# kkromberg/SpeechRecognition

Measured on AMD Instinct MI355X. Metric: frames/sec scored+decoded, higher is better.
Workload: dtype f64

## Files before the change

### include/srgpu.h

```cpp
#ifndef SRGPU_H
#define SRGPU_H

#include <stddef.h>
#include <stdint.h>

#ifdef __cplusplus
extern "C" {
#endif

#if defined(__GNUC__)
#define SR_API __attribute__((visibility("default")))
#else
#define SR_API
#endif

#define SR_ABI_VERSION 4
SR_API int sr_abi_version(void);

#define SR_OK 0
#define SR_EINVAL (-1)
#define SR_EHIP (-2)
#define SR_ENODEV (-3)
#define SR_ELIMIT (-4)
#define SR_ENOMEM (-5)
// ... 263 lines not shown
                                 sr_bigram_stream** out);
SR_API int sr_bigram_stream_begin(sr_bigram_stream* s, uint32_t* id);
SR_API int sr_bigram_stream_push(sr_bigram_stream* s, uint32_t n, const uint32_t* ids, const float* feats, const uint64_t* frame_off);
SR_API int sr_bigram_stream_partial(sr_bigram_stream* s, uint32_t id, uint32_t* out_word, float* out_score, uint32_t* out_time,
                                    uint32_t cap, uint32_t* count, uint64_t* frames);
SR_API int sr_bigram_stream_end(sr_bigram_stream* s, uint32_t id, uint32_t* out_word, float* out_score, uint32_t* out_time,
                                uint32_t cap, uint32_t* count);
SR_API int sr_bigram_stream_destroy(sr_bigram_stream* s);

SR_API int sr_probe_fp16_denormals(int device, int* preserved);
SR_API int sr_probe_fp16_accumulation(int device, int* within_model, double* worst_ratio);

SR_API int sr_prefilter_masks(sr_model* m, const float* feats, uint64_t n_frames, int route, uint32_t* n_groups, uint32_t* masks,
                              uint64_t cap_words);
SR_API int sr_prefilter_range_frames(uint32_t* frames);

typedef struct {
  double gmm_ms;
  uint64_t gmm_launches;
  double gmm_flops;
  double search_ms;
  uint64_t search_launches;
  double search_bytes;
  uint64_t frames;
  uint64_t refined_pairs;
  uint64_t refined_densities;
  double prefilter_ms;
  double refine_ms;
} sr_profile;
SR_API int sr_profile_enable(sr_model* m, int on);
// ... 8 lines not shown
```

### speechrecognition_amd/build.py

```python
from __future__ import annotations

import hashlib
import os
import subprocess
import sys

HERE = os.path.dirname(os.path.abspath(__file__))
CSRC = os.path.join(HERE, "csrc")
LIB = os.path.join(HERE, "libsrgpu.so")
SOURCES = ["srgpu_api.cpp", "mixset.cpp", "feeder.cpp", "gmm_mfma.hip", "gmm_exact.hip", "gmm_prefilter.hip", "viterbi_decode.hip",
           "viterbi_fast.hip", "viterbi_words.hip", "viterbi_align.hip", "viterbi_fb.hip", "viterbi_netfb.hip", "viterbi_mmi.hip", "viterbi_smbr.hip", "viterbi_lattice.hip", "viterbi_bigram.hip", "viterbi_bigram_fb.hip", "viterbi_bigram_mmi.hip", "viterbi_bigram_smbr.hip", "viterbi_bigram_lattice.hip", "posterior_items.hip",
           "em_accumulate.hip", "em_finalize.hip", "fmllr_stats.hip", "fmllr.cpp", "mllr_stats.hip", "mllt_stats.hip", "lda_stats.hip", "model_structure.hip"]
HEADERS = ["mllr.cpp", "mllt.cpp", "lda.cpp", "kernels.h", "host_util.h", "handles.h", "traceback.h", "dpp_util.h", "netfb_device.h", "smbr_device.h", "sym_contract.h", "structure_plan.h", "fb_plan.h", os.path.join("..", "..", "include", "srgpu.h")]
FLAGS = ["-O3", "-std=c++17", "--offload-arch=gfx950", "-fPIC", "-fvisibility=hidden", "-Wall", "-Wno-unused-function"]
PER_FILE = {"gmm_exact.hip": ["-ffp-contract=off"], "gmm_prefilter.hip": ["-ffp-contract=off"], "em_accumulate.hip": ["-ffp-contract=off"],
            "em_finalize.hip": ["-ffp-contract=off"],
            "viterbi_bigram_lattice.hip": ["-ffp-contract=off"],
            "fmllr_stats.hip": ["-ffp-contract=off"],
            "mllr_stats.hip": ["-ffp-contract=off"],
            "mllt_stats.hip": ["-ffp-contract=off"],
            "lda_stats.hip": ["-ffp-contract=off"],
            "model_structure.hip": ["-ffp-contract=off"]}
MAX_PARALLEL = 8


def _read(path):
    with open(path, "rb") as f:
# ... 115 lines not shown
```

### speechrecognition_amd/capi.py

```python
from __future__ import annotations

import ctypes as C
import os

import numpy as np

HERE = os.path.dirname(os.path.abspath(__file__))
LIB_PATH = os.environ.get("SRGPU_LIB") or os.path.join(HERE, "libsrgpu.so")

GMM_MFMA, GMM_EXACT, GMM_PREFILTER, GMM_DEFAULT = 0, 1, 2, 3
POOL_GLOBAL, POOL_MIXTURE, POOL_NONE = 0, 1, 2
SEARCH_GENERAL_KERNEL = 1
SEARCH_SLOT_KERNEL = 2
BIGRAM_DENSE_STATES = 1
BIGRAM_GLOBAL_STATES = 2
SR_ECORRUPT = -7
LDA_SKIP = 0xFFFFFFFF
SR_ABI_VERSION = 4

SYMBOLS = [
    "sr_abi_version", "sr_model_trim",
    "sr_last_error", "sr_device_count", "sr_model_create", "sr_model_load_mixset", "sr_model_destroy", "sr_model_info",
    "sr_corpus_upload", "sr_corpus_upload_async", "sr_corpus_wait", "sr_corpus_destroy", "sr_shard_utterances", "sr_recognize_batch_multi", "sr_score_corpus", "sr_score_frames", "sr_lexicon_create",
    "sr_lexicon_destroy", "sr_lexicon_describe", "sr_recognize_corpus", "sr_traceback_corpus", "sr_traceback_words", "sr_recognize_batch", "sr_align_corpus", "sr_align_corpus_pruned", "sr_path_scores_corpus", "sr_model_create_from_statistics", "sr_model_create_from_accumulated", "sr_mixset_write", "sr_model_set_tying", "sr_model_tying_info", "sr_model_topology", "sr_accumulate_corpus",
# ... 3 lines not shown
    "sr_smbr_max_positions", "sr_net_accuracies_corpus", "sr_smbr_statistics_corpus",
    "sr_word_lattice_corpus", "sr_lattice_nbest",
    "sr_fmllr_statistics_corpus", "sr_fmllr_statistics_bw_corpus", "sr_fmllr_estimate", "sr_corpus_transform",
    "sr_mllr_statistics_corpus", "sr_mllr_statistics_bw_corpus", "sr_mllr_estimate", "sr_model_transform_means",
    "sr_mllt_statistics_corpus", "sr_mllt_statistics_bw_corpus", "sr_mllt_estimate",
    "sr_lda_statistics_corpus", "sr_lda_estimate", "sr_corpus_splice_transform",
    "sr_bigram_create", "sr_bigram_destroy", "sr_bigram_describe", "sr_recognize_bigram_corpus",
    "sr_bigram_word_posteriors_corpus", "sr_recognize_bigram_confidence_corpus",
    "sr_bigram_occupancies_corpus", "sr_bigram_mmi_statistics_corpus",
    "sr_bigram_accuracies_corpus", "sr_bigram_smbr_statistics_corpus",
    "sr_bigram_word_lattice_corpus", "sr_bigram_lattice_nbest",
    "sr_stream_open", "sr_stream_begin", "sr_stream_push", "sr_stream_partial", "sr_stream_end", "sr_stream_destroy",
    "sr_bigram_stream_open", "sr_bigram_stream_begin", "sr_bigram_stream_push", "sr_bigram_stream_partial", "sr_bigram_stream_end",
    "sr_bigram_stream_destroy",
    "sr_probe_fp16_denormals", "sr_probe_fp16_accumulation", "sr_prefilter_masks", "sr_prefilter_range_frames",
    "sr_profile_enable", "sr_profile_reset", "sr_profile_read",
]


class SrError(RuntimeError):
    def __init__(self, code, msg):
        super().__init__(f"libsrgpu error {code}: {msg}")
        self.code = code


def prefilter_range_frames():
    n = C.c_uint32()
    _check(lib().sr_prefilter_range_frames(C.byref(n)))
    return n.value

# ... 109 lines not shown
        L.sr_stream_begin.argtypes = [vp, C.POINTER(u32)]
        L.sr_stream_push.argtypes = [vp, u32, vp, vp, vp]
        L.sr_stream_partial.argtypes = [vp, u32, vp, u32, C.POINTER(u32), C.POINTER(u64)]
        L.sr_stream_end.argtypes = [vp, u32, vp, u32, C.POINTER(u32), vp, vp, vp]
        L.sr_stream_destroy.argtypes = [vp]
        L.sr_bigram_stream_open.argtypes = [vp, vp, C.POINTER(BigramParams), u32, u64, C.POINTER(vp)]
        L.sr_bigram_stream_begin.argtypes = [vp, C.POINTER(u32)]
        L.sr_bigram_stream_push.argtypes = [vp, u32, vp, vp, vp]
        L.sr_bigram_stream_partial.argtypes = [vp, u32, vp, vp, vp, u32, C.POINTER(u32), C.POINTER(u64)]
        L.sr_bigram_stream_end.argtypes = [vp, u32, vp, vp, vp, u32, C.POINTER(u32)]
        L.sr_bigram_stream_destroy.argtypes = [vp]
        L.sr_probe_fp16_denormals.argtypes = [i32, C.POINTER(i32)]
        L.sr_probe_fp16_accumulation.argtypes = [i32, C.POINTER(i32), C.POINTER(dbl)]
        L.sr_prefilter_masks.argtypes = [vp, vp, u64, i32, C.POINTER(u32), vp, u64]
        L.sr_prefilter_range_frames.argtypes = [C.POINTER(u32)]
        L.sr_profile_enable.argtypes = [vp, i32]
        L.sr_profile_reset.argtypes = [vp]
        L.sr_profile_read.argtypes = [vp, C.POINTER(Profile)]
        _lib = L
    return _lib


def _check(rc):
    if rc != 0:
        raise SrError(rc, lib().sr_last_error().decode(errors="replace"))


def device_count():
    n = C.c_int(0)
    _check(lib().sr_device_count(C.byref(n)))
# ... 112 lines not shown
        self.close()

    def score_frames(self, feats, kernel=GMM_PREFILTER):
        feats = np.ascontiguousarray(feats, dtype=np.float32)
        out = np.empty((feats.shape[0], self.n_states), dtype=np.float64)
        _check(lib().sr_score_frames(self.h, _ptr(feats), feats.shape[0], kernel, _ptr(out)))
        return out

    def prefilter_masks(self, feats, route):
        feats = np.ascontiguousarray(feats, dtype=np.float32)
        n_groups = C.c_uint32()
        _check(lib().sr_prefilter_masks(self.h, None, feats.shape[0], route, C.byref(n_groups), None, 0))
        out = np.empty((n_groups.value, feats.shape[0], 4), dtype=np.uint32)
        _check(lib().sr_prefilter_masks(self.h, _ptr(feats), feats.shape[0], route, C.byref(n_groups), _ptr(out), out.size))
        return out

    def upload(self, feats, frame_off, asynchronous=False):
        return Corpus(self, feats, frame_off, asynchronous)

    def recognize_batch(self, lexicon, feats, frame_off, am_threshold, word_penalty, kernel=GMM_PREFILTER):
        feats = np.ascontiguousarray(feats, dtype=np.float32)
        frame_off = np.ascontiguousarray(frame_off, dtype=np.uint64)
        n = len(frame_off) - 1
        words = np.zeros(max(int(frame_off[-1]), 1), dtype=np.uint32)
        woff = np.zeros(n + 1, dtype=np.uint64)
        sp = SearchParams(am_threshold, word_penalty, kernel, 0)
        _check(lib().sr_recognize_batch(self.h, lexicon.h, C.byref(sp), _ptr(feats), _ptr(frame_off), n, _ptr(words), _ptr(woff)))
        return words[: int(woff[-1])].copy(), woff

    def lexicon(self, word_off, automaton, silence_idx, tdp, silence_state):
# ... 728 lines not shown
```

### speechrecognition_amd/csrc/handles.h

```cpp
#pragma once
#include <hip/hip_runtime.h>

#include <atomic>
#include <condition_variable>
#include <cstdint>
#include <map>
#include <memory>
#include <mutex>
#include <string>
#include <thread>
#include <vector>

#include "../../include/srgpu.h"
#include "host_util.h"
#include "kernels.h"

namespace srhost {
int fail(int code, const char* fmt, ...) __attribute__((format(printf, 2, 3)));
}

#define HIP_TRY(expr)                                                                             \
  do {                                                                                            \
    hipError_t e_ = (expr);                                                                       \
    if (e_ != hipSuccess) return srhost::fail(SR_EHIP, "%s: %s (%s:%d)", #expr, hipGetErrorString(e_), __FILE__, __LINE__); \
// ... 12 lines not shown
    return e;
  }
  hipError_t upload(const T* src, size_t count) {
    hipError_t e = ensure(count);
    if (e != hipSuccess || count == 0) return e;
    return hipMemcpy(p, src, count * sizeof(T), hipMemcpyHostToDevice);
  }
  void release() { if (p) (void)hipFree(p); p = nullptr; n = 0; }
  void swap(DevBuf& o) { T* tp = p; p = o.p; o.p = tp; size_t tn = n; n = o.n; o.n = tn; }
  DevBuf() = default;
  DevBuf(const DevBuf&) = delete;
  DevBuf& operator=(const DevBuf&) = delete;
  ~DevBuf() { release(); }
};

struct EventPair { hipEvent_t a, b; int kind; };


struct sr_feeder;


struct CorpusSpare {
  DevBuf<float> feats;
  DevBuf<uint64_t> d_frame_off;
  DevBuf<uint32_t> utt_order, out_words, out_count, out_flags;
  DevBuf<double> tb_score;
  DevBuf<uint16_t> tb_word, tb_bkp;
  size_t bytes() const {
    return feats.n * 4 + d_frame_off.n * 8 + (utt_order.n + out_words.n + out_count.n + out_flags.n) * 4 + tb_score.n * 8 + (tb_word.n + tb_bkp.n) * 2;
  }
};
size_t corpus_spare_cap_bytes();

struct sr_model {
  int device = 0;
  uint32_t dim = 0, n_states = 0, ld = 0;
  uint64_t n_dens = 0;
  bool max_approx = true;
  DevBuf<uint32_t> dens_off;
  DevBuf<double> means, inv_vars, norm, logw;
  DevBuf<uint32_t> dens_mean, dens_var;
  std::vector<uint32_t> h_dens_off, h_dens_mean, h_dens_var;
  std::vector<double> h_means, h_inv_vars, h_norm, h_logw;
  bool mfma_packed = false, pf_packed = false;
// ... 6 lines not shown
  std::map<uint32_t, std::unique_ptr<DevBuf<uint32_t>>> split_tabs, pf_split_tabs;
  const uint32_t *split_cur = nullptr, *pf_split_cur = nullptr;
  uint32_t split_ny = 0;
  int pf_ks32 = 0;
  uint32_t pf_groups = 0, pf_ny = 0, max_dens = 0, pf_slots = 0, pf_chunks = 1, pf_pstates = 0;
  DevBuf<unsigned char> pf_apack;
  DevBuf<float> pf_lim, featsT, featsP;
  DevBuf<uint4> pf_defer;
  DevBuf<uint32_t> pf_defer_cnt;
  int neg_possible = -1;
  uint32_t pf_dp = 0;
  DevBuf<uint32_t> pf_mask, pf_ndens, pf_ring;
  DevBuf<uint4> pf_bfrag;
  DevBuf<float2> pf_bnorm;
  int pf_route = srgpu::kPfStationary;
  DevBuf<double> pf_rows;
  DevBuf<unsigned long long> pf_counter;
  hipStream_t s_copy = nullptr;
  float* staging[2] = {nullptr, nullptr};
  hipEvent_t staging_free[2] = {nullptr, nullptr};
  std::atomic<bool> staging_busy{false};
  std::mutex spare_mu;
  std::unique_ptr<CorpusSpare> spare;
  std::vector<sr_corpus*> corpora;
  hipStream_t s_gmm = nullptr, s_search = nullptr;
  DevBuf<double> scores[2];
  hipEvent_t ev_scored[2] = {nullptr, nullptr}, ev_consumed[2] = {nullptr, nullptr};
  size_t chunk_frames = 0;
  bool overlap = true;
  size_t defer_budget = (size_t)32 << 30;
// ... 7 lines not shown
};

struct sr_corpus {
  sr_model* model = nullptr;
  sr_feeder* feeder = nullptr;
  uint32_t n_utts = 0;
  uint64_t n_frames = 0;
  std::vector<uint64_t> frame_off;
  DevBuf<float> feats;
  DevBuf<uint64_t> d_frame_off;
  DevBuf<uint32_t> utt_order;
  size_t order_chunk_frames = 0;
  DevBuf<double> tb_score;
  DevBuf<uint16_t> tb_word, tb_bkp;
  DevBuf<uint32_t> out_words, out_count, out_flags;
  DevBuf<unsigned char> big_ws;
  DevBuf<uint16_t> automata, out_states;
  DevBuf<uint64_t> aut_off, bp_off, al_blk_frame0;
  DevBuf<uint32_t> al_list_off, al_states, al_blk_frames, al_blk_list;
  DevBuf<uint8_t> backptr;
  DevBuf<double> out_cost, path_scores;
  DevBuf<uint64_t> pair_off;
  DevBuf<uint32_t> pair_frame, key_mean, key_var, iota, keys_sorted, pairs_sorted, row_begin;
  DevBuf<double> pair_w, acc_mean, acc_var, w_mean, w_var;
  bool acc_valid = false;
  uint32_t acc_n_mean = 0, acc_n_var = 0;
  DevBuf<unsigned char> sort_temp;
  DevBuf<double> fb_trellis, fb_item_w, fb_weight;
  DevBuf<uint64_t> fb_trellis_off, fb_pair_cnt, fb_pair_end;
  DevBuf<uint32_t> fb_mix_off, fb_slot_beg, fb_cnt, fb_scan, fb_base, fb_item_off, fb_item_frame;
// ... 144 lines not shown
```

### speechrecognition_amd/csrc/kernels.h

```cpp
#pragma once
#include <hip/hip_runtime.h>
#include <stdint.h>

#include <vector>

namespace srgpu {

struct GmmMfmaArgs {
  const float* feats;
  uint64_t n_frames;
  uint32_t dim;
  const double* apack;
  const uint32_t* blk_meta;
  const uint32_t* grp_state;
  const uint32_t* split_begin;
  double* out;
  uint32_t ld;
  uint32_t nx, ny;
};
int gmm_mfma_ksteps_for_dim(uint32_t dim);
int gmm_mfma_frames_per_tile(int ksteps);
hipError_t launch_gmm_mfma(const GmmMfmaArgs& a, int ksteps, bool sum, hipStream_t stream);

struct GmmExactArgs {
// ... 175 lines not shown
  const StreamJob* jobs;
  unsigned char* ws;
  size_t ws_stride;
  StreamState* state;
  double* tb_score;
  uint16_t* tb_word;
  uint16_t* tb_bkp;
  uint64_t tb_stride;
  uint32_t* words;
  uint64_t words_stride;
};
hipError_t launch_decode_stream(const StreamArgs& a, uint32_t n_jobs, hipStream_t stream);
hipError_t launch_traceback(const uint64_t* frame_off, uint32_t n_utts, const uint16_t* tb_word, const uint16_t* tb_bkp,
                            uint32_t silence_word, uint32_t n_words, uint32_t* out_words, uint32_t* out_count,
                            uint32_t* out_flags, hipStream_t stream);

struct AlignArgs {
  const double* scores;
  uint32_t ld;
  const uint64_t* frame_off;
  uint64_t frame_base;
  uint32_t utt_first, n_utts;
  const uint32_t* utt_order;
  const uint16_t* automata;
  const uint64_t* aut_off;
  double tdp_loop, tdp_forward, tdp_skip;
  uint32_t silence_state;
  double pruning_threshold;
  uint8_t* backptr;
  const uint64_t* bp_off;
// ... 447 lines not shown
```

### speechrecognition_amd/csrc/srgpu_api.cpp

```cpp
#include <hip/hip_runtime.h>

#include <algorithm>
#include <cmath>
#include <cstdarg>
#include <cstdio>
#include <cstdlib>
#include <cstring>
#include <limits>
#include <map>
#include <memory>
#include <mutex>
#include <numeric>
#include <queue>
#include <set>
#include <string>
#include <vector>

#include "../../include/srgpu.h"
#include "fb_plan.h"
#include "host_util.h"
#include "kernels.h"
#include "traceback.h"

using namespace srgpu;
// ... 493 lines not shown
    if ((rc = launch_scoring(m, c->feats.p + a * m->dim, cuts[i] - a, gmm_kernel, table + (a - f0) * m->ld))) return rc;
    a = cuts[i];
  }
  return SR_OK;
}

int prepare_chunks(sr_model* m, sr_corpus* c, std::vector<Chunk>* chunks) {
  *chunks = make_chunks(c, m->chunk_frames);
  uint64_t mx = 0;
  for (const Chunk& ch : *chunks) mx = std::max(mx, ch.f1 - ch.f0);
  const int nbuf = chunks->size() > 1 ? 2 : 1;
  for (int i = 0; i < nbuf; i++) HIP_TRY(m->scores[i].ensure((size_t)mx * m->ld));
  return ensure_utt_order(m, c, *chunks);
}

template <class Score, class Search>
int run_chunks(sr_model* m, const std::vector<Chunk>& chunks, Score score, Search search) {
  const hipStream_t s_search = m->overlap ? m->s_search : m->s_gmm;
  int rc;
  for (size_t i = 0; i < chunks.size(); i++) {
    const int buf = (int)(i & 1);
    if (i >= 2) HIP_TRY(hipStreamWaitEvent(m->s_gmm, m->ev_consumed[buf], 0));
    if ((rc = score(chunks[i], m->scores[buf].p))) return rc;
    HIP_TRY(hipEventRecord(m->ev_scored[buf], m->s_gmm));
    HIP_TRY(hipStreamWaitEvent(s_search, m->ev_scored[buf], 0));
    EventPair ep{};
    if ((rc = prof_begin(m, s_search, 1, &ep))) return rc;
    if ((rc = search(chunks[i], m->scores[buf].p, s_search))) return rc;
    if ((rc = prof_end(m, s_search, &ep))) return rc;
    HIP_TRY(hipEventRecord(m->ev_consumed[buf], s_search));
  }
  HIP_TRY(hipStreamSynchronize(m->s_search));
  HIP_TRY(hipStreamSynchronize(m->s_gmm));
  return SR_OK;
}

}
namespace srhost {
static void swap_spare(sr_corpus* c, CorpusSpare& sp) {
  c->feats.swap(sp.feats); c->d_frame_off.swap(sp.d_frame_off); c->utt_order.swap(sp.utt_order); c->out_words.swap(sp.out_words);
  c->out_count.swap(sp.out_count); c->out_flags.swap(sp.out_flags); c->tb_score.swap(sp.tb_score); c->tb_word.swap(sp.tb_word);
  c->tb_bkp.swap(sp.tb_bkp);
}
void corpus_register(sr_corpus* c) {
  sr_model* m = c->model;
  std::lock_guard<std::mutex> lk(m->spare_mu);
  m->corpora.push_back(c);
}
void corpus_adopt_spare(sr_corpus* c) {
  sr_model* m = c->model;
  std::unique_ptr<CorpusSpare> sp;
  { std::lock_guard<std::mutex> lk(m->spare_mu); sp = std::move(m->spare); }
  if (sp) swap_spare(c, *sp);
  c->order_chunk_frames = 0;
}
size_t corpus_spare_cap_bytes() {
  static const size_t cap = [] {
    const char* e = getenv("SRGPU_SPARE_MB");
    const long mb = e ? atol(e) : 256;
    return (size_t)(mb < 0 ? 0 : mb) << 20;
  }();
  return cap;
}
void corpus_donate_spare(sr_corpus* c) {
  sr_model* m = c->model;
  if (!m) return;
  std::unique_ptr<CorpusSpare> sp(new CorpusSpare());
  swap_spare(c, *sp);
  std::lock_guard<std::mutex> lk(m->spare_mu);
  m->corpora.erase(std::remove(m->corpora.begin(), m->corpora.end(), c), m->corpora.end());
  if (sp->bytes() > corpus_spare_cap_bytes()) return;
  if (!m->spare) m->spare = std::move(sp);
}
}
namespace {

int check_model(const sr_model* m) {
  if (!m) return fail(SR_EINVAL, "null model handle");
  HIP_TRY(hipSetDevice(m->device));
  return SR_OK;
}
int check_corpus(const sr_model* m, const sr_corpus* c) {
  int rc = check_model(m);
  if (rc) return rc;
  if (!c || c->model != m) return fail(SR_EINVAL, "corpus does not belong to this model");
  return SR_OK;
// ... 126 lines not shown
  const char* env = getenv("SRGPU_SCORE_CHUNK_MB");
  size_t chunk_bytes = (size_t)49152 << 20;
  {
    size_t free_b = 0, total_b = 0;
    if (hipMemGetInfo(&free_b, &total_b) == hipSuccess && total_b) chunk_bytes = std::min(chunk_bytes, total_b / 6);
  }
  if (env) chunk_bytes = (size_t)atol(env) << 20;
  m->chunk_frames = std::max<size_t>(1, chunk_bytes / ((size_t)m->ld * sizeof(double)));
  m->chunk_frames = std::min<size_t>(m->chunk_frames, ((size_t)1 << 32) / (4 * (size_t)dim) - 128);
  if (const char* ov = getenv("SRGPU_OVERLAP")) m->overlap = atoi(ov) != 0;
  if (const char* e = getenv("SRGPU_PREFILTER")) {
    if (!strcmp(e, "staged")) m->pf_route = kPfStaged;
    else if (!strcmp(e, "stationary")) m->pf_route = kPfStationary;
    else return fail(SR_EINVAL, "SRGPU_PREFILTER=%s: staged or stationary", e);
  }
  if (const char* e = getenv("SRGPU_DEFER_MB")) m->defer_budget = (size_t)strtoull(e, nullptr, 10) << 20;
  if (const char* e = getenv("SRGPU_FB_MB")) m->fb_budget = std::max<size_t>(1, (size_t)strtoull(e, nullptr, 10)) << 20;
  if (const char* e = getenv("SRGPU_MLLT_MB")) m->mllt_budget = std::max<size_t>(1, (size_t)strtoull(e, nullptr, 10)) << 20;
  if (const char* e = getenv("SRGPU_LDA_MB")) m->lda_budget = std::max<size_t>(1, (size_t)strtoull(e, nullptr, 10)) << 20;
  if (const char* e = getenv("SRGPU_DEFER_CAP")) m->defer_cap_limit = std::max(1u, (uint32_t)strtoul(e, nullptr, 10));
  *out = own.release();
  return SR_OK;
}

int ensure_host_tables(sr_model* m) {
  const size_t C = m->n_dens, D = m->dim;
  if (m->h_norm.size() == C && m->h_means.size() == C * D) return SR_OK;
  m->h_means.resize(C * D); m->h_inv_vars.resize(C * D); m->h_norm.resize(C); m->h_logw.resize(C);
  if (C == 0) return SR_OK;
  HIP_TRY(hipMemcpy(m->h_means.data(), m->means.p, C * D * sizeof(double), hipMemcpyDeviceToHost));
// ... 313 lines not shown
  else if (r.big) snprintf(out, cap, "big (%u positions: hypotheses in device memory)", l->net.n_slots);
  else snprintf(out, cap, "slots (%u type-padded positions)", l->fast.n_slots);
  return SR_OK;
  });
}

int sr_lexicon_destroy(sr_lexicon* l) {
  return guarded(__func__, [&]() -> int {
  if (!l) return SR_OK;
  if (l->model) { (void)hipSetDevice(l->model->device); (void)hipDeviceSynchronize(); }
  delete l;
  return SR_OK;
  });
}

static int gather_words(sr_corpus* c, uint32_t* out_words, uint64_t* out_word_off) {
  const uint32_t U = c->n_utts;
  const uint64_t F = c->n_frames;
  std::vector<uint32_t> counts(U), flags(U), dev_words(F);
  if (U) HIP_TRY(hipMemcpy(counts.data(), c->out_count.p, sizeof(uint32_t) * U, hipMemcpyDeviceToHost));
  if (U) HIP_TRY(hipMemcpy(flags.data(), c->out_flags.p, sizeof(uint32_t) * U, hipMemcpyDeviceToHost));
  if (F) HIP_TRY(hipMemcpy(dev_words.data(), c->out_words.p, sizeof(uint32_t) * F, hipMemcpyDeviceToHost));
  uint64_t w = 0;
  out_word_off[0] = 0;
  for (uint32_t u = 0; u < U; u++) {
    if (flags[u] & kFlagCorrupt) return fail(SR_ECORRUPT, "utterance %u: the traceback does not walk back to frame 0 (Recognizer.cpp:222-231)", u);
    const uint64_t b = c->frame_off[u], T = c->frame_off[u + 1] - b;
    if (counts[u] > T) return fail(SR_ECORRUPT, "utterance %u: %u words for %llu frames", u, counts[u], (unsigned long long)T);
    for (uint32_t i = 0; i < counts[u]; i++) out_words[w++] = dev_words[b + i];
    out_word_off[u + 1] = w;
  }
  return SR_OK;
}

extern "C++" {
template <class After>
static int recognize_pass(sr_model* m, sr_corpus* c, sr_lexicon* l, const sr_search_params* p, const std::vector<Chunk>& chunks,
                          After after) {
  const uint32_t U = c->n_utts;
  const uint64_t F = c->n_frames;
  HIP_TRY(c->tb_score.ensure(F + U));
  HIP_TRY(c->tb_word.ensure(F + U));
  HIP_TRY(c->tb_bkp.ensure(F + U));
  HIP_TRY(c->out_words.ensure(F));
  HIP_TRY(c->out_count.ensure(U));
  HIP_TRY(c->out_flags.ensure(U));
  HIP_TRY(hipMemsetAsync(c->out_flags.p, 0, sizeof(uint32_t) * std::max(1u, U), m->s_gmm));

  DecodeArgs da = lexicon_args(l);
  da.frame_off = c->d_frame_off.p; da.utt_order = c->utt_order.p;
  da.am_threshold = p->am_threshold; da.word_penalty = p->word_penalty;
  if (p->flags & ~(SR_SEARCH_GENERAL_KERNEL | SR_SEARCH_SLOT_KERNEL)) return fail(SR_EINVAL, "unknown sr_search_params.flags 0x%x", (unsigned)p->flags);
  const DecodeRoute route = decode_route(da, p->flags & SR_SEARCH_GENERAL_KERNEL, p->flags & SR_SEARCH_SLOT_KERNEL);
  if (route.big) {
    uint32_t most = 0;
    for (const Chunk& ch : chunks) most = std::max(most, ch.u1 - ch.u0);
    HIP_TRY(c->big_ws.ensure((size_t)most * decode_big_workspace(l->net.n_slots)));
  }
  int rc;
  {
    bool neg = false;
    if ((rc = srhost::may_go_negative(m, &neg))) return rc;
    da.exact_negative = neg ? 1u : 0u;
  }
  da.tb_score = c->tb_score.p; da.tb_word = c->tb_word.p; da.tb_bkp = c->tb_bkp.p;
  da.out_words = c->out_words.p; da.out_count = c->out_count.p; da.out_flags = c->out_flags.p;

  rc = run_chunks(m, chunks, [&](const Chunk& ch, double* table) { return score_chunk(m, c, ch.f0, ch.f1, p->gmm_kernel, table); },
      [&](const Chunk& ch, const double* table, hipStream_t s) -> int {
        da.scores = table; da.frame_base = ch.f0; da.utt_first = ch.u0; da.n_utts = ch.u1 - ch.u0;
        HIP_TRY(launch_decode(da, route, c->big_ws.p, s));
        if (m->profiling) m->prof.search_bytes += (8.0 * m->n_states + 4.0 * l->net.n_slots) * (double)(ch.f1 - ch.f0);
        return after(ch, table, s);
      });
  if (rc) return rc;
  if (m->profiling) m->prof.frames += F;
  return SR_OK;
}
}

int sr_recognize_corpus(sr_model* m, sr_corpus* c, sr_lexicon* l, const sr_search_params* p, uint32_t* out_words,
                        uint64_t* out_word_off, double* tb_score, uint16_t* tb_word, uint16_t* tb_bkp) {
  return guarded(__func__, [&]() -> int {
  int rc = check_corpus(m, c);
  if (rc) return rc;
  if (!l || l->model != m) return fail(SR_EINVAL, "lexicon does not belong to this model");
  if (!p || !out_word_off || (!out_words && c->n_frames)) return fail(SR_EINVAL, "null argument");
  const uint32_t U = c->n_utts;
  const uint64_t F = c->n_frames;
// ... 10 lines not shown

int sr_traceback_corpus(sr_model* m, sr_corpus* c, sr_lexicon* l, const uint16_t* tb_word, const uint16_t* tb_bkp,
                        uint32_t* out_words, uint64_t* out_word_off) {
  return guarded(__func__, [&]() -> int {
  int rc = check_corpus(m, c);
  if (rc) return rc;
  if (!l || l->model != m) return fail(SR_EINVAL, "lexicon does not belong to this model");
  if (!tb_word || !tb_bkp || !out_word_off || (!out_words && c->n_frames)) return fail(SR_EINVAL, "null argument");
  const uint32_t U = c->n_utts;
  const uint64_t F = c->n_frames;
  HIP_TRY(c->tb_word.ensure(F + U));
  HIP_TRY(c->tb_bkp.ensure(F + U));
  HIP_TRY(c->out_words.ensure(F));
  HIP_TRY(c->out_count.ensure(U));
  HIP_TRY(c->out_flags.ensure(U));
  HIP_TRY(hipMemcpyAsync(c->tb_word.p, tb_word, sizeof(uint16_t) * (F + U), hipMemcpyHostToDevice, m->s_gmm));
  HIP_TRY(hipMemcpyAsync(c->tb_bkp.p, tb_bkp, sizeof(uint16_t) * (F + U), hipMemcpyHostToDevice, m->s_gmm));
  HIP_TRY(launch_traceback(c->d_frame_off.p, U, c->tb_word.p, c->tb_bkp.p, l->net.silence_word, l->net.n_words, c->out_words.p,
                           c->out_count.p, c->out_flags.p, m->s_gmm));
  HIP_TRY(hipStreamSynchronize(m->s_gmm));
  return gather_words(c, out_words, out_word_off);
  });
}

int sr_traceback_words(uint32_t n_frames, const uint16_t* tb_word, const uint16_t* tb_bkp, uint32_t silence_word, uint32_t n_words,
                       uint32_t* out_words, uint32_t* out_count) {
  return guarded(__func__, [&]() -> int {
  if (!tb_word || !tb_bkp || !out_count || (!out_words && n_frames)) return fail(SR_EINVAL, "null argument");
  *out_count = 0;
  const uint32_t n = walk_traceback(
      n_frames, silence_word, n_words, [&](uint32_t t) -> uint32_t { return tb_word[t]; },
      [&](uint32_t t) -> uint32_t { return tb_bkp[t]; }, out_words, n_frames);
  if (n == kTbCorrupt) return fail(SR_ECORRUPT, "not a traceback: a back pointer that does not fall, or a word outside the lexicon");
  *out_count = n;
  return SR_OK;
  });
// ... 81 lines not shown
  const uint64_t per_frame = p->max_word_ends ? std::min<uint64_t>(p->max_word_ends, W) : W;
  std::vector<uint64_t> book_off(U + 1, 0);
  uint32_t max_chunk_utts = 0;
  for (uint32_t u = 0; u < U; u++) book_off[u + 1] = book_off[u] + 2 + per_frame * (c->frame_off[u + 1] - c->frame_off[u]);
  for (const Chunk& ch : chunks) max_chunk_utts = std::max(max_chunk_utts, ch.u1 - ch.u0);
  HIP_TRY(b->book.ensure(book_off[U]));
  HIP_TRY(b->book_off.upload(book_off.data(), book_off.size()));
  HIP_TRY(b->we_slot.ensure((size_t)max_chunk_utts * 4 * W));
  HIP_TRY(b->we_bp.ensure((size_t)max_chunk_utts * 4 * W));
  HIP_TRY(b->we_score.ensure((size_t)max_chunk_utts * 4 * W));
  HIP_TRY(b->out_word.ensure(F + U));
  HIP_TRY(b->out_time.ensure(F + U));
  HIP_TRY(b->out_score.ensure(F + U));
  HIP_TRY(b->out_count.ensure(U));
  HIP_TRY(b->out_flags.ensure(U));

  ba.frame_off = c->d_frame_off.p; ba.utt_order = c->utt_order.p;
  ba.ac_pruning = p->acoustic_pruning; ba.lm_pruning = p->lm_pruning;
  if (layout == BigramLayout::kGlobal) {
    int dev_cus = 0;
    HIP_TRY(hipDeviceGetAttribute(&dev_cus, hipDeviceAttributeMultiprocessorCount, m->device));
    const uint64_t per_wg = bigram_gs_ws_words(W, ba.n_positions);
    size_t free_b = 0, total_b = 0;
    HIP_TRY(hipMemGetInfo(&free_b, &total_b));
    const uint64_t have = b->gs_ws.n / per_wg;
    const uint64_t cap = std::max<uint64_t>(have, (free_b / 4) / (per_wg * 4));
    const uint64_t grid = std::min<uint64_t>({(uint64_t)std::max(dev_cus, 1) * 2, (uint64_t)std::max(max_chunk_utts, 1u), cap});
    if (grid == 0) return fail(SR_ENOMEM, "bigram search: %llu bytes of device memory for one state image, %zu free",
                                (unsigned long long)(per_wg * 4), free_b);
    HIP_TRY(b->gs_ws.ensure(grid * per_wg));
// ... 4 lines not shown
      HIP_TRY(hipDeviceSynchronize());
      ba.gs_active = b->gs_active.p;
    }
  }
  ba.we_slot = b->we_slot.p; ba.we_bp = b->we_bp.p; ba.we_score = b->we_score.p;
  ba.book = b->book.p; ba.book_off = b->book_off.p;
  ba.out_word = b->out_word.p; ba.out_score = b->out_score.p; ba.out_time = b->out_time.p;
  ba.out_count = b->out_count.p; ba.out_flags = b->out_flags.p;

  rc = run_chunks(m, chunks, [&](const Chunk& ch, double* table) { return score_chunk(m, c, ch.f0, ch.f1, p->gmm_kernel, table); },
      [&](const Chunk& ch, const double* table, hipStream_t s) -> int {
        ba.scores = table; ba.frame_base = ch.f0; ba.utt_first = ch.u0; ba.n_utts = ch.u1 - ch.u0;
        HIP_TRY(launch_bigram(ba, s));
        if (m->profiling) m->prof.search_bytes += (8.0 * m->n_states + 4.0 * ba.n_positions) * (double)(ch.f1 - ch.f0);
        return after(ch, table, s);
      });
  if (rc) return rc;

  std::vector<uint32_t> counts(U), flags(U), dw(F + U), dt(F + U);
  std::vector<float> ds(F + U);
  if (U) {
    HIP_TRY(hipMemcpy(counts.data(), b->out_count.p, sizeof(uint32_t) * U, hipMemcpyDeviceToHost));
    HIP_TRY(hipMemcpy(flags.data(), b->out_flags.p, sizeof(uint32_t) * U, hipMemcpyDeviceToHost));
    HIP_TRY(hipMemcpy(dw.data(), b->out_word.p, sizeof(uint32_t) * (F + U), hipMemcpyDeviceToHost));
    HIP_TRY(hipMemcpy(dt.data(), b->out_time.p, sizeof(uint32_t) * (F + U), hipMemcpyDeviceToHost));
    HIP_TRY(hipMemcpy(ds.data(), b->out_score.p, sizeof(float) * (F + U), hipMemcpyDeviceToHost));
  }
  uint64_t n = 0;
  out_off[0] = 0;
  for (uint32_t u = 0; u < U; u++) {
    if (flags[u]) return fail(SR_ELIMIT, "utterance %u: more than %llu word ends per frame (sr_bigram_params.max_word_ends)", u,
                              (unsigned long long)per_frame);
    const uint64_t o = c->frame_off[u] + u;
    for (uint32_t i = 0; i < counts[u]; i++, n++) { out_word[n] = dw[o + i]; out_score[n] = ds[o + i]; out_time[n] = dt[o + i]; }
    out_off[u + 1] = n;
  }
  if (ba.gs_active) {
    unsigned long long visited = 0;
    HIP_TRY(hipMemcpy(&visited, ba.gs_active, sizeof visited, hipMemcpyDeviceToHost));
    fprintf(stderr, "srgpu bigram: global states, %llu frames, %.1f active positions per frame\n", (unsigned long long)F,
            F ? (double)visited / (double)F : 0.0);
  }
  if (m->profiling) m->prof.frames += F;
  return SR_OK;
}
}

int sr_recognize_bigram_corpus(sr_model* m, sr_corpus* c, sr_bigram* b, const sr_bigram_params* p, uint32_t* out_word,
                               float* out_score, uint32_t* out_time, uint64_t* out_off) {
  return guarded(__func__, [&]() -> int {
// ... 3015 lines not shown
```

Before: 13.94 million.

## Compact decoded words on device into mapped pinned buffer instead of host gather

Adds a device gather step: a single-block scan kernel computes per-utterance output offsets and error flags, then a copy kernel compacts the word, time and score arrays into a mapped, coherent pinned host block. It is enqueued at the end of the chunk pipeline, so the host only memcpys the already-compact result. This replaces several full-size synchronous device-to-host copies and the host-side per-utterance loop. In exchange it adds two launches and a serial single-block scan, and the copy kernel writes over PCIe into host memory.

```diff
diff --git a/include/srgpu.h b/include/srgpu.h
--- a/include/srgpu.h
+++ b/include/srgpu.h
@@ -301,6 +301,8 @@
 SR_API int sr_prefilter_masks(sr_model* m, const float* feats, uint64_t n_frames, int route, uint32_t* n_groups, uint32_t* masks,
                               uint64_t cap_words);
 SR_API int sr_prefilter_range_frames(uint32_t* frames);
+SR_API int sr_gather_words(sr_model* m, uint32_t n_utts, const uint64_t* frame_off, const uint32_t* counts, const uint32_t* flags,
+                           const uint32_t* words, uint32_t* out_words, uint64_t* out_word_off);
 
 typedef struct {
   double gmm_ms;
diff --git a/speechrecognition_amd/build.py b/speechrecognition_amd/build.py
--- a/speechrecognition_amd/build.py
+++ b/speechrecognition_amd/build.py
@@ -10,7 +10,8 @@
 LIB = os.path.join(HERE, "libsrgpu.so")
 SOURCES = ["srgpu_api.cpp", "mixset.cpp", "feeder.cpp", "gmm_mfma.hip", "gmm_exact.hip", "gmm_prefilter.hip", "viterbi_decode.hip",
            "viterbi_fast.hip", "viterbi_words.hip", "viterbi_align.hip", "viterbi_fb.hip", "viterbi_netfb.hip", "viterbi_mmi.hip", "viterbi_smbr.hip", "viterbi_lattice.hip", "viterbi_bigram.hip", "viterbi_bigram_fb.hip", "viterbi_bigram_mmi.hip", "viterbi_bigram_smbr.hip", "viterbi_bigram_lattice.hip", "posterior_items.hip",
-           "em_accumulate.hip", "em_finalize.hip", "fmllr_stats.hip", "fmllr.cpp", "mllr_stats.hip", "mllt_stats.hip", "lda_stats.hip", "model_structure.hip"]
+           "em_accumulate.hip", "em_finalize.hip", "fmllr_stats.hip", "fmllr.cpp", "mllr_stats.hip", "mllt_stats.hip", "lda_stats.hip", "model_structure.hip",
+           "gather_words.hip"]
 HEADERS = ["mllr.cpp", "mllt.cpp", "lda.cpp", "kernels.h", "host_util.h", "handles.h", "traceback.h", "dpp_util.h", "netfb_device.h", "smbr_device.h", "sym_contract.h", "structure_plan.h", "fb_plan.h", os.path.join("..", "..", "include", "srgpu.h")]
 FLAGS = ["-O3", "-std=c++17", "--offload-arch=gfx950", "-fPIC", "-fvisibility=hidden", "-Wall", "-Wno-unused-function"]
 PER_FILE = {"gmm_exact.hip": ["-ffp-contract=off"], "gmm_prefilter.hip": ["-ffp-contract=off"], "em_accumulate.hip": ["-ffp-contract=off"],
diff --git a/speechrecognition_amd/capi.py b/speechrecognition_amd/capi.py
--- a/speechrecognition_amd/capi.py
+++ b/speechrecognition_amd/capi.py
@@ -41,6 +41,7 @@
     "sr_bigram_stream_open", "sr_bigram_stream_begin", "sr_bigram_stream_push", "sr_bigram_stream_partial", "sr_bigram_stream_end",
     "sr_bigram_stream_destroy",
     "sr_probe_fp16_denormals", "sr_probe_fp16_accumulation", "sr_prefilter_masks", "sr_prefilter_range_frames",
+    "sr_gather_words",
     "sr_profile_enable", "sr_profile_reset", "sr_profile_read",
 ]
 
@@ -180,6 +181,7 @@
         L.sr_probe_fp16_accumulation.argtypes = [i32, C.POINTER(i32), C.POINTER(dbl)]
         L.sr_prefilter_masks.argtypes = [vp, vp, u64, i32, C.POINTER(u32), vp, u64]
         L.sr_prefilter_range_frames.argtypes = [C.POINTER(u32)]
+        L.sr_gather_words.argtypes = [vp, u32, vp, vp, vp, vp, vp, vp]
         L.sr_profile_enable.argtypes = [vp, i32]
         L.sr_profile_reset.argtypes = [vp]
         L.sr_profile_read.argtypes = [vp, C.POINTER(Profile)]
@@ -322,6 +324,18 @@
         out = np.empty((n_groups.value, feats.shape[0], 4), dtype=np.uint32)
         _check(lib().sr_prefilter_masks(self.h, _ptr(feats), feats.shape[0], route, C.byref(n_groups), _ptr(out), out.size))
         return out
+
+    def gather_words(self, frame_off, counts, flags, words):
+        frame_off = np.ascontiguousarray(frame_off, dtype=np.uint64)
+        counts = np.ascontiguousarray(counts, dtype=np.uint32)
+        flags = np.ascontiguousarray(flags, dtype=np.uint32)
+        words = np.ascontiguousarray(words, dtype=np.uint32)
+        n_utts = len(frame_off) - 1
+        assert len(counts) == n_utts and len(flags) == n_utts and len(words) == int(frame_off[-1])
+        out = np.empty(max(1, len(words)), dtype=np.uint32)
+        off = np.empty(n_utts + 1, dtype=np.uint64)
+        _check(lib().sr_gather_words(self.h, n_utts, _ptr(frame_off), _ptr(counts), _ptr(flags), _ptr(words), _ptr(out), _ptr(off)))
+        return out[:int(off[-1])].copy(), off
 
     def upload(self, feats, frame_off, asynchronous=False):
         return Corpus(self, feats, frame_off, asynchronous)
diff --git a/speechrecognition_amd/csrc/gather_words.hip b/speechrecognition_amd/csrc/gather_words.hip
--- /dev/null
+++ b/speechrecognition_amd/csrc/gather_words.hip
@@ -0,0 +1,110 @@
+#include <hip/hip_runtime.h>
+
+#include "kernels.h"
+
+namespace srgpu {
+
+constexpr uint32_t kScanThreads = 1024, kScanWaves = kScanThreads / 64;
+constexpr uint32_t kCopyThreads = 256;
+constexpr uint32_t kCopyGroup = 8;
+
+static __device__ inline uint64_t* block_off(const GatherArgs& a) { return reinterpret_cast<uint64_t*>(a.block + sizeof(GatherHeader)); }
+
+__global__ __launch_bounds__(kScanThreads) void gather_scan_kernel(GatherArgs a) {
+  __shared__ unsigned long long wave_sum[kScanWaves];
+  __shared__ uint32_t first_flagged, first_over;
+  const uint32_t tid = threadIdx.x, lane = tid & 63u, wave = tid >> 6;
+  if (tid == 0) { first_flagged = kGatherNone; first_over = kGatherNone; }
+  uint64_t* off = block_off(a);
+  unsigned long long carry = 0;
+  uint32_t my_flagged = kGatherNone, my_over = kGatherNone, my_over_count = 0;
+  for (uint32_t base = 0; base < a.n_utts; base += kScanThreads) {
+    const uint32_t u = base + tid;
+    const bool live = u < a.n_utts;
+    uint32_t n = 0;
+    if (live) {
+      const uint64_t slots = a.frame_off[u + 1] - a.frame_off[u] + a.extra_slots;
+      n = a.count[u];
+      if ((a.flags[u] & a.flag_mask) && my_flagged == kGatherNone) my_flagged = u;
+      if (n > slots) {
+        if (my_over == kGatherNone) { my_over = u; my_over_count = n; }
+        n = (uint32_t)slots;
+      }
+    }
+    unsigned long long x = n;
+    for (uint32_t d = 1; d < 64; d <<= 1) {
+      const unsigned long long y = __shfl_up(x, d, 64);
+      if (lane >= d) x += y;
+    }
+    if (lane == 63) wave_sum[wave] = x;
+    __syncthreads();
+    unsigned long long before = 0, tile = 0;
+    for (uint32_t w = 0; w < kScanWaves; w++) {
+      const unsigned long long s = wave_sum[w];
+      if (w < wave) before += s;
+      tile += s;
+    }
+    __syncthreads();
+    if (live) {
+      const uint64_t end = carry + before + x;
+      a.dev_off[u + 1] = end;
+      off[u + 1] = end;
+    }
+    carry += tile;
+  }
+  __syncthreads();
+  if (my_flagged != kGatherNone) atomicMin(&first_flagged, my_flagged);
+  if (my_over != kGatherNone) atomicMin(&first_over, my_over);
+  __syncthreads();
+  GatherHeader* h = reinterpret_cast<GatherHeader*>(a.block);
+  if (my_over != kGatherNone && my_over == first_over) h->over_count = my_over_count;
+  if (tid == 0) {
+    h->n_words = carry;
+    h->first_flagged = first_flagged;
+    h->first_over = first_over;
+    if (first_over == kGatherNone) h->over_count = 0;
+    a.dev_off[0] = 0;
+    off[0] = 0;
+  }
+}
+
+template <int N>
+__global__ __launch_bounds__(kCopyThreads) void gather_copy_kernel(GatherArgs a) {
+  __shared__ uint64_t s_off[kCopyGroup + 1], s_src[kCopyGroup];
+  const uint32_t tid = threadIdx.x;
+  const uint32_t u0 = blockIdx.x * kCopyGroup, nu = min(kCopyGroup, a.n_utts - u0);
+  if (tid <= nu) s_off[tid] = a.dev_off[u0 + tid];
+  if (tid < nu) s_src[tid] = a.frame_off[u0 + tid] + (uint64_t)(u0 + tid) * a.extra_slots;
+  __syncthreads();
+  const uint64_t total = a.dev_off[a.n_utts];
+  uint32_t* dst = reinterpret_cast<uint32_t*>(block_off(a) + a.n_utts + 1);
+  const uint64_t hi = s_off[nu];
+  for (uint64_t j = s_off[0] + tid; j < hi; j += kCopyThreads) {
+    uint32_t i = 0;
+    for (uint32_t step = kCopyGroup / 2; step; step >>= 1)
+      if (i + step < nu && s_off[i + step] <= j) i += step;
+    const uint64_t s = s_src[i] + (j - s_off[i]);
+#pragma unroll
+    for (int k = 0; k < N; k++) dst[(uint64_t)k * total + j] = a.src[k][s];
+  }
+}
+
+size_t gather_block_bytes(uint32_t n_utts, uint64_t n_slots, int n_arrays) {
+  return sizeof(GatherHeader) + sizeof(uint64_t) * ((size_t)n_utts + 1) + sizeof(uint32_t) * (size_t)n_slots * (size_t)n_arrays;
+}
+
+hipError_t launch_gather_words(const GatherArgs& a, int n_arrays, hipStream_t stream) {
+  if (n_arrays < 1 || n_arrays > kGatherMaxArrays || !a.block || !a.dev_off) return hipErrorInvalidValue;
+  hipLaunchKernelGGL(gather_scan_kernel, dim3(1), dim3(kScanThreads), 0, stream, a);
+  hipError_t e = hipGetLastError();
+  if (e != hipSuccess || a.n_utts == 0) return e;
+  const dim3 grid((a.n_utts + kCopyGroup - 1) / kCopyGroup), block(kCopyThreads);
+  switch (n_arrays) {
+    case 1: hipLaunchKernelGGL(gather_copy_kernel<1>, grid, block, 0, stream, a); break;
+    case 2: hipLaunchKernelGGL(gather_copy_kernel<2>, grid, block, 0, stream, a); break;
+    default: hipLaunchKernelGGL(gather_copy_kernel<3>, grid, block, 0, stream, a); break;
+  }
+  return hipGetLastError();
+}
+
+}
diff --git a/speechrecognition_amd/csrc/handles.h b/speechrecognition_amd/csrc/handles.h
--- a/speechrecognition_amd/csrc/handles.h
+++ b/speechrecognition_amd/csrc/handles.h
@@ -50,6 +50,26 @@
   ~DevBuf() { release(); }
 };
 
+template <typename T>
+struct PinnedBuf {
+  T* p = nullptr;
+  size_t n = 0;
+  hipError_t ensure(size_t count) {
+    if (count <= n && p) return hipSuccess;
+    if (p) { hipError_t e = hipHostFree(p); if (e != hipSuccess) return e; p = nullptr; n = 0; }
+    if (count == 0) count = 1;
+    hipError_t e = hipHostMalloc(reinterpret_cast<void**>(&p), count * sizeof(T), hipHostMallocMapped | hipHostMallocCoherent);
+    if (e == hipSuccess) n = count;
+    return e;
+  }
+  void release() { if (p) (void)hipHostFree(p); p = nullptr; n = 0; }
+  void swap(PinnedBuf& o) { T* tp = p; p = o.p; o.p = tp; size_t tn = n; n = o.n; o.n = tn; }
+  PinnedBuf() = default;
+  PinnedBuf(const PinnedBuf&) = delete;
+  PinnedBuf& operator=(const PinnedBuf&) = delete;
+  ~PinnedBuf() { release(); }
+};
+
 struct EventPair { hipEvent_t a, b; int kind; };
 
 
@@ -62,8 +82,11 @@
   DevBuf<uint32_t> utt_order, out_words, out_count, out_flags;
   DevBuf<double> tb_score;
   DevBuf<uint16_t> tb_word, tb_bkp;
+  DevBuf<uint64_t> gather_off;
+  PinnedBuf<unsigned char> result;
   size_t bytes() const {
-    return feats.n * 4 + d_frame_off.n * 8 + (utt_order.n + out_words.n + out_count.n + out_flags.n) * 4 + tb_score.n * 8 + (tb_word.n + tb_bkp.n) * 2;
+    return feats.n * 4 + d_frame_off.n * 8 + (utt_order.n + out_words.n + out_count.n + out_flags.n) * 4 + tb_score.n * 8 + (tb_word.n + tb_bkp.n) * 2 +
+           gather_off.n * 8 + result.n;
   }
 };
 size_t corpus_spare_cap_bytes();
@@ -100,6 +123,7 @@
   DevBuf<uint4> pf_bfrag;
   DevBuf<float2> pf_bnorm;
   int pf_route = srgpu::kPfStationary;
+  bool gather_device = true;
   DevBuf<double> pf_rows;
   DevBuf<unsigned long long> pf_counter;
   hipStream_t s_copy = nullptr;
@@ -137,6 +161,8 @@
   DevBuf<double> tb_score;
   DevBuf<uint16_t> tb_word, tb_bkp;
   DevBuf<uint32_t> out_words, out_count, out_flags;
+  PinnedBuf<unsigned char> result;
+  DevBuf<uint64_t> gather_off;
   DevBuf<unsigned char> big_ws;
   DevBuf<uint16_t> automata, out_states;
   DevBuf<uint64_t> aut_off, bp_off, al_blk_frame0;
diff --git a/speechrecognition_amd/csrc/kernels.h b/speechrecognition_amd/csrc/kernels.h
--- a/speechrecognition_amd/csrc/kernels.h
+++ b/speechrecognition_amd/csrc/kernels.h
@@ -213,6 +213,28 @@
 hipError_t launch_traceback(const uint64_t* frame_off, uint32_t n_utts, const uint16_t* tb_word, const uint16_t* tb_bkp,
                             uint32_t silence_word, uint32_t n_words, uint32_t* out_words, uint32_t* out_count,
                             uint32_t* out_flags, hipStream_t stream);
+
+constexpr uint32_t kGatherNone = 0xFFFFFFFFu;
+constexpr int kGatherMaxArrays = 3;
+struct GatherHeader {
+  uint64_t n_words;
+  uint32_t first_flagged;
+  uint32_t first_over;
+  uint32_t over_count;
+  uint32_t reserved[3];
+};
+static_assert(sizeof(GatherHeader) == 32, "word_off follows the header, 8-byte aligned");
+struct GatherArgs {
+  const uint32_t* count;
+  const uint32_t* flags;
+  const uint64_t* frame_off;
+  uint32_t n_utts, extra_slots, flag_mask;
+  const uint32_t* src[kGatherMaxArrays];
+  uint64_t* dev_off;
+  unsigned char* block;
+};
+size_t gather_block_bytes(uint32_t n_utts, uint64_t n_slots, int n_arrays);
+hipError_t launch_gather_words(const GatherArgs& a, int n_arrays, hipStream_t stream);
 
 struct AlignArgs {
   const double* scores;
diff --git a/speechrecognition_amd/csrc/srgpu_api.cpp b/speechrecognition_amd/csrc/srgpu_api.cpp
--- a/speechrecognition_amd/csrc/srgpu_api.cpp
+++ b/speechrecognition_amd/csrc/srgpu_api.cpp
@@ -531,8 +531,8 @@
   return ensure_utt_order(m, c, *chunks);
 }
 
-template <class Score, class Search>
-int run_chunks(sr_model* m, const std::vector<Chunk>& chunks, Score score, Search search) {
+template <class Score, class Search, class Tail>
+int run_chunks(sr_model* m, const std::vector<Chunk>& chunks, Score score, Search search, Tail tail) {
   const hipStream_t s_search = m->overlap ? m->s_search : m->s_gmm;
   int rc;
   for (size_t i = 0; i < chunks.size(); i++) {
@@ -547,9 +547,14 @@
     if ((rc = prof_end(m, s_search, &ep))) return rc;
     HIP_TRY(hipEventRecord(m->ev_consumed[buf], s_search));
   }
+  if ((rc = tail(s_search))) return rc;
   HIP_TRY(hipStreamSynchronize(m->s_search));
   HIP_TRY(hipStreamSynchronize(m->s_gmm));
   return SR_OK;
+}
+template <class Score, class Search>
+int run_chunks(sr_model* m, const std::vector<Chunk>& chunks, Score score, Search search) {
+  return run_chunks(m, chunks, score, search, [](hipStream_t) { return (int)SR_OK; });
 }
 
 }
@@ -557,7 +562,7 @@
 static void swap_spare(sr_corpus* c, CorpusSpare& sp) {
   c->feats.swap(sp.feats); c->d_frame_off.swap(sp.d_frame_off); c->utt_order.swap(sp.utt_order); c->out_words.swap(sp.out_words);
   c->out_count.swap(sp.out_count); c->out_flags.swap(sp.out_flags); c->tb_score.swap(sp.tb_score); c->tb_word.swap(sp.tb_word);
-  c->tb_bkp.swap(sp.tb_bkp);
+  c->tb_bkp.swap(sp.tb_bkp); c->gather_off.swap(sp.gather_off); c->result.swap(sp.result);
 }
 void corpus_register(sr_corpus* c) {
   sr_model* m = c->model;
@@ -586,7 +591,12 @@
   swap_spare(c, *sp);
   std::lock_guard<std::mutex> lk(m->spare_mu);
   m->corpora.erase(std::remove(m->corpora.begin(), m->corpora.end(), c), m->corpora.end());
-  if (sp->bytes() > corpus_spare_cap_bytes()) return;
+  if (sp->bytes() > corpus_spare_cap_bytes()) {
+    std::unique_ptr<CorpusSpare> small(new CorpusSpare());
+    small->result.swap(sp->result); small->gather_off.swap(sp->gather_off);
+    sp = std::move(small);
+    if (sp->bytes() > corpus_spare_cap_bytes()) return;
+  }
   if (!m->spare) m->spare = std::move(sp);
 }
 }
@@ -743,6 +753,11 @@
     else if (!strcmp(e, "stationary")) m->pf_route = kPfStationary;
     else return fail(SR_EINVAL, "SRGPU_PREFILTER=%s: staged or stationary", e);
   }
+  if (const char* e = getenv("SRGPU_GATHER")) {
+    if (!strcmp(e, "host")) m->gather_device = false;
+    else if (!strcmp(e, "device")) m->gather_device = true;
+    else return fail(SR_EINVAL, "SRGPU_GATHER=%s: host or device", e);
+  }
   if (const char* e = getenv("SRGPU_DEFER_MB")) m->defer_budget = (size_t)strtoull(e, nullptr, 10) << 20;
   if (const char* e = getenv("SRGPU_FB_MB")) m->fb_budget = std::max<size_t>(1, (size_t)strtoull(e, nullptr, 10)) << 20;
   if (const char* e = getenv("SRGPU_MLLT_MB")) m->mllt_budget = std::max<size_t>(1, (size_t)strtoull(e, nullptr, 10)) << 20;
@@ -1086,7 +1101,51 @@
   });
 }
 
+static int reserve_gather(sr_model* m, sr_corpus* c, uint32_t extra_slots, int n_arrays) {
+  if (!m->gather_device) return SR_OK;
+  HIP_TRY(c->result.ensure(gather_block_bytes(c->n_utts, c->n_frames + (uint64_t)c->n_utts * extra_slots, n_arrays)));
+  HIP_TRY(c->gather_off.ensure((size_t)c->n_utts + 1));
+  return SR_OK;
+}
+static int enqueue_gather(sr_model* m, sr_corpus* c, GatherArgs a, int n_arrays, hipStream_t s) {
+  if (!m->gather_device) return SR_OK;
+  a.frame_off = c->d_frame_off.p; a.n_utts = c->n_utts;
+  a.dev_off = c->gather_off.p; a.block = c->result.p;
+  HIP_TRY(launch_gather_words(a, n_arrays, s));
+  return SR_OK;
+}
+static GatherArgs zerogram_gather(const sr_corpus* c) {
+  GatherArgs a{};
+  a.count = c->out_count.p; a.flags = c->out_flags.p; a.flag_mask = kFlagCorrupt; a.extra_slots = 0;
+  a.src[0] = c->out_words.p;
+  return a;
+}
+struct GatherBlock {
+  const GatherHeader* head;
+  const uint64_t* off;
+  const uint32_t* data;
+};
+static GatherBlock gather_block(const sr_corpus* c) {
+  const uint64_t* off = reinterpret_cast<const uint64_t*>(c->result.p + sizeof(GatherHeader));
+  return {reinterpret_cast<const GatherHeader*>(c->result.p), off, reinterpret_cast<const uint32_t*>(off + c->n_utts + 1)};
+}
+
+static int gather_words_host(sr_corpus* c, uint32_t* out_words, uint64_t* out_word_off);
 static int gather_words(sr_corpus* c, uint32_t* out_words, uint64_t* out_word_off) {
+  if (!c->model->gather_device) return gather_words_host(c, out_words, out_word_off);
+  const GatherBlock b = gather_block(c);
+  const GatherHeader& h = *b.head;
+  if (h.first_flagged != kGatherNone && h.first_flagged <= h.first_over)
+    return fail(SR_ECORRUPT, "utterance %u: the traceback does not walk back to frame 0 (Recognizer.cpp:222-231)", h.first_flagged);
+  if (h.first_over != kGatherNone) {
+    const uint64_t T = c->frame_off[h.first_over + 1] - c->frame_off[h.first_over];
+    return fail(SR_ECORRUPT, "utterance %u: %u words for %llu frames", h.first_over, h.over_count, (unsigned long long)T);
+  }
+  memcpy(out_word_off, b.off, sizeof(uint64_t) * ((size_t)c->n_utts + 1));
+  if (h.n_words) memcpy(out_words, b.data, sizeof(uint32_t) * h.n_words);
+  return SR_OK;
+}
+static int gather_words_host(sr_corpus* c, uint32_t* out_words, uint64_t* out_word_off) {
   const uint32_t U = c->n_utts;
   const uint64_t F = c->n_frames;
   std::vector<uint32_t> counts(U), flags(U), dev_words(F);
@@ -1117,6 +1176,8 @@
   HIP_TRY(c->out_words.ensure(F));
   HIP_TRY(c->out_count.ensure(U));
   HIP_TRY(c->out_flags.ensure(U));
+  int rc;
+  if ((rc = reserve_gather(m, c, 0, 1))) return rc;
   HIP_TRY(hipMemsetAsync(c->out_flags.p, 0, sizeof(uint32_t) * std::max(1u, U), m->s_gmm));
 
   DecodeArgs da = lexicon_args(l);
@@ -1129,7 +1190,6 @@
     for (const Chunk& ch : chunks) most = std::max(most, ch.u1 - ch.u0);
     HIP_TRY(c->big_ws.ensure((size_t)most * decode_big_workspace(l->net.n_slots)));
   }
-  int rc;
   {
     bool neg = false;
     if ((rc = srhost::may_go_negative(m, &neg))) return rc;
@@ -1144,7 +1204,8 @@
         HIP_TRY(launch_decode(da, route, c->big_ws.p, s));
         if (m->profiling) m->prof.search_bytes += (8.0 * m->n_states + 4.0 * l->net.n_slots) * (double)(ch.f1 - ch.f0);
         return after(ch, table, s);
-      });
+      },
+      [&](hipStream_t s) { return enqueue_gather(m, c, zerogram_gather(c), 1, s); });
   if (rc) return rc;
   if (m->profiling) m->prof.frames += F;
   return SR_OK;
@@ -1185,12 +1246,38 @@
   HIP_TRY(c->out_words.ensure(F));
   HIP_TRY(c->out_count.ensure(U));
   HIP_TRY(c->out_flags.ensure(U));
+  if ((rc = reserve_gather(m, c, 0, 1))) return rc;
   HIP_TRY(hipMemcpyAsync(c->tb_word.p, tb_word, sizeof(uint16_t) * (F + U), hipMemcpyHostToDevice, m->s_gmm));
   HIP_TRY(hipMemcpyAsync(c->tb_bkp.p, tb_bkp, sizeof(uint16_t) * (F + U), hipMemcpyHostToDevice, m->s_gmm));
   HIP_TRY(launch_traceback(c->d_frame_off.p, U, c->tb_word.p, c->tb_bkp.p, l->net.silence_word, l->net.n_words, c->out_words.p,
                            c->out_count.p, c->out_flags.p, m->s_gmm));
+  if ((rc = enqueue_gather(m, c, zerogram_gather(c), 1, m->s_gmm))) return rc;
   HIP_TRY(hipStreamSynchronize(m->s_gmm));
   return gather_words(c, out_words, out_word_off);
+  });
+}
+
+int sr_gather_words(sr_model* m, uint32_t n_utts, const uint64_t* frame_off, const uint32_t* counts, const uint32_t* flags,
+                    const uint32_t* words, uint32_t* out_words, uint64_t* out_word_off) {
+  return guarded(__func__, [&]() -> int {
+  int rc = check_model(m);
+  if (rc) return rc;
+  if (!frame_off || !out_word_off || (n_utts && (!counts || !flags))) return fail(SR_EINVAL, "null argument");
+  if (frame_off[0] != 0) return fail(SR_EINVAL, "frame_off[0] must be 0");
+  for (uint32_t u = 0; u < n_utts; u++)
+    if (frame_off[u + 1] < frame_off[u]) return fail(SR_EINVAL, "frame_off falls at utterance %u", u);
+  sr_corpus c;
+  c.model = m; c.n_utts = n_utts; c.n_frames = frame_off[n_utts];
+  if (c.n_frames && (!words || !out_words)) return fail(SR_EINVAL, "null argument");
+  c.frame_off.assign(frame_off, frame_off + n_utts + 1);
+  HIP_TRY(c.d_frame_off.upload(frame_off, (size_t)n_utts + 1));
+  HIP_TRY(c.out_count.upload(counts, n_utts));
+  HIP_TRY(c.out_flags.upload(flags, n_utts));
+  HIP_TRY(c.out_words.upload(words, c.n_frames));
+  if ((rc = reserve_gather(m, &c, 0, 1))) return rc;
+  if ((rc = enqueue_gather(m, &c, zerogram_gather(&c), 1, m->s_gmm))) return rc;
+  HIP_TRY(hipStreamSynchronize(m->s_gmm));
+  return gather_words(&c, out_words, out_word_off);
   });
 }
 
@@ -1302,6 +1389,7 @@
   HIP_TRY(b->out_score.ensure(F + U));
   HIP_TRY(b->out_count.ensure(U));
   HIP_TRY(b->out_flags.ensure(U));
+  if ((rc = reserve_gather(m, c, 1, 3))) return rc;
 
   ba.frame_off = c->d_frame_off.p; ba.utt_order = c->utt_order.p;
   ba.ac_pruning = p->acoustic_pruning; ba.lm_pruning = p->lm_pruning;
@@ -1336,26 +1424,47 @@
         HIP_TRY(launch_bigram(ba, s));
         if (m->profiling) m->prof.search_bytes += (8.0 * m->n_states + 4.0 * ba.n_positions) * (double)(ch.f1 - ch.f0);
         return after(ch, table, s);
+      },
+      [&](hipStream_t s) {
+        GatherArgs ga{};
+        ga.count = b->out_count.p; ga.flags = b->out_flags.p; ga.flag_mask = ~0u; ga.extra_slots = 1;
+        ga.src[0] = b->out_word.p; ga.src[1] = b->out_time.p; ga.src[2] = reinterpret_cast<const uint32_t*>(b->out_score.p);
+        return enqueue_gather(m, c, ga, 3, s);
       });
   if (rc) return rc;
 
-  std::vector<uint32_t> counts(U), flags(U), dw(F + U), dt(F + U);
-  std::vector<float> ds(F + U);
-  if (U) {
-    HIP_TRY(hipMemcpy(counts.data(), b->out_count.p, sizeof(uint32_t) * U, hipMemcpyDeviceToHost));
-    HIP_TRY(hipMemcpy(flags.data(), b->out_flags.p, sizeof(uint32_t) * U, hipMemcpyDeviceToHost));
-    HIP_TRY(hipMemcpy(dw.data(), b->out_word.p, sizeof(uint32_t) * (F + U), hipMemcpyDeviceToHost));
-    HIP_TRY(hipMemcpy(dt.data(), b->out_time.p, sizeof(uint32_t) * (F + U), hipMemcpyDeviceToHost));
-    HIP_TRY(hipMemcpy(ds.data(), b->out_score.p, sizeof(float) * (F + U), hipMemcpyDeviceToHost));
-  }
-  uint64_t n = 0;
-  out_off[0] = 0;
-  for (uint32_t u = 0; u < U; u++) {
-    if (flags[u]) return fail(SR_ELIMIT, "utterance %u: more than %llu word ends per frame (sr_bigram_params.max_word_ends)", u,
-                              (unsigned long long)per_frame);
-    const uint64_t o = c->frame_off[u] + u;
-    for (uint32_t i = 0; i < counts[u]; i++, n++) { out_word[n] = dw[o + i]; out_score[n] = ds[o + i]; out_time[n] = dt[o + i]; }
-    out_off[u + 1] = n;
+  if (m->gather_device) {
+    const GatherBlock g = gather_block(c);
+    const GatherHeader& h = *g.head;
+    if (h.first_flagged != kGatherNone && h.first_flagged <= h.first_over)
+      return fail(SR_ELIMIT, "utterance %u: more than %llu word ends per frame (sr_bigram_params.max_word_ends)", h.first_flagged,
+                  (unsigned long long)per_frame);
+    if (h.first_over != kGatherNone) return fail(SR_ECORRUPT, "utterance %u: %u entries for its frames", h.first_over, h.over_count);
+    memcpy(out_off, g.off, sizeof(uint64_t) * ((size_t)U + 1));
+    if (h.n_words) {
+      memcpy(out_word, g.data, sizeof(uint32_t) * h.n_words);
+      memcpy(out_time, g.data + h.n_words, sizeof(uint32_t) * h.n_words);
+      memcpy(out_score, g.data + 2 * h.n_words, sizeof(float) * h.n_words);
+    }
+  } else {
+    std::vector<uint32_t> counts(U), flags(U), dw(F + U), dt(F + U);
+    std::vector<float> ds(F + U);
+    if (U) {
+      HIP_TRY(hipMemcpy(counts.data(), b->out_count.p, sizeof(uint32_t) * U, hipMemcpyDeviceToHost));
+      HIP_TRY(hipMemcpy(flags.data(), b->out_flags.p, sizeof(uint32_t) * U, hipMemcpyDeviceToHost));
+      HIP_TRY(hipMemcpy(dw.data(), b->out_word.p, sizeof(uint32_t) * (F + U), hipMemcpyDeviceToHost));
+      HIP_TRY(hipMemcpy(dt.data(), b->out_time.p, sizeof(uint32_t) * (F + U), hipMemcpyDeviceToHost));
+      HIP_TRY(hipMemcpy(ds.data(), b->out_score.p, sizeof(float) * (F + U), hipMemcpyDeviceToHost));
+    }
+    uint64_t n = 0;
+    out_off[0] = 0;
+    for (uint32_t u = 0; u < U; u++) {
+      if (flags[u]) return fail(SR_ELIMIT, "utterance %u: more than %llu word ends per frame (sr_bigram_params.max_word_ends)", u,
+                                (unsigned long long)per_frame);
+      const uint64_t o = c->frame_off[u] + u;
+      for (uint32_t i = 0; i < counts[u]; i++, n++) { out_word[n] = dw[o + i]; out_score[n] = ds[o + i]; out_time[n] = dt[o + i]; }
+      out_off[u + 1] = n;
+    }
   }
   if (ba.gs_active) {
     unsigned long long visited = 0;
```

Result: faster. 14.10 million (median of 6 runs) (+1.2%).
